# ArtyZe/yolo_quantization

Hardware: AMD Instinct MI355X
Metric: images/sec yolov3-tiny INT8 416x416 (higher is better)
Workload: dtype u8 x s8 -> int32 (f64 or exact-integer requant, bit-identical)

## Files before the change

### include/mi355_yolo_int8.h

```cpp
#ifndef MI355_YOLO_INT8_H
#define MI355_YOLO_INT8_H
#include <stddef.h>
#include <stdint.h>

#ifdef __cplusplus
extern "C" {
#endif

#define MI355_OK 0
#define MI355_EINVAL (-22)
#define MI355_ENOMEM (-12)
#define MI355_EHIP (-5)
#define MI355_ENODEV (-19)

#define MI355_ACT_RELU 1
#define MI355_ACT_LINEAR 3
#define MI355_ACT_RELU6 8
#define MI355_ACT_LEAKY 9

#define MI355_STORE_WRAP 0
#define MI355_STORE_SATURATE 1

#define MI355_ACC_EXACT 0
#define MI355_ACC_REF_F32 1
// ... 38 lines not shown
    int tail;
} mi355_tensor;

size_t mi355_tensor_describe(mi355_tensor *t, int B, int H, int W, int C);
size_t mi355_tensor_describe_nchw(mi355_tensor *t, int B, int H, int W, int C);
int mi355_tensor_fill(const mi355_tensor *t, uint8_t zero_point, void *stream);
int mi355_nchw_to_tensor(const uint8_t *nchw, const mi355_tensor *t, void *stream);
int mi355_tensor_to_nchw(const mi355_tensor *t, uint8_t *nchw, void *stream);

size_t mi355_conv_pack_size(int n, int c, int ksize);
int mi355_conv_pack(int n, int c, int ksize, const uint8_t *weights_uint8, const uint8_t *zp_w,
                    const int32_t *biases_int32, const double *M_value, const double *shift_value, void *blob);
int mi355_conv_pack_epilogue(int n, int c, int ksize, int activation, int zp_act, void *blob);

typedef struct mi355_conv_desc {
    int n, c, ksize, stride, pad;
    int activation;
    int store_mode;
    int accum_mode;
    uint8_t zp_in, zp_act;
    float s_act;
    int plan;
    int epilogue_packed;
} mi355_conv_desc;
#define MI355_PLAN_LATENCY 0
#define MI355_PLAN_THROUGHPUT 1

int mi355_conv_forward(const mi355_conv_desc *desc, const mi355_tensor *x, const void *blob, const uint8_t *w_u8,
                       const uint8_t *zp_w, const mi355_tensor *y, int32_t *acc_out, float *y_f32, void *stream);

int mi355_conv_pool_forward(const mi355_conv_desc *desc, const mi355_tensor *x, const void *blob, const mi355_tensor *y,
                            const mi355_tensor *ypool, void *stream);

int mi355_conv_yolo_forward(const mi355_conv_desc *desc, const mi355_tensor *x, const void *blob, const mi355_tensor *y,
                            float *y_f32, float *yolo_out, int classes, void *stream);

int mi355_conv_upsample_forward(const mi355_conv_desc *desc, const mi355_tensor *x, const void *blob, const mi355_tensor *y_up,
                                int stride, void *stream);

int mi355_conv_shortcut_forward(const mi355_conv_desc *desc, const mi355_tensor *x, const void *blob, const mi355_tensor *from,
                                const mi355_tensor *y_sum, int32_t Ka, int32_t Kb, uint8_t zp_from, uint8_t zp_out, void *stream);

int mi355_conv_forward_per_image(const mi355_conv_desc *desc, const mi355_tensor *x, const void *bank, size_t entry_bytes,
                                 const int32_t *entry_of_image, const uint8_t *zp_in_of_image, const uint8_t *w_u8,
                                 const uint8_t *zp_w, const mi355_tensor *y, int32_t *acc_out, float *y_f32, void *stream);
int mi355_conv_pool_forward_per_image(const mi355_conv_desc *desc, const mi355_tensor *x, const void *bank, size_t entry_bytes,
                                      const int32_t *entry_of_image, const uint8_t *zp_in_of_image, const mi355_tensor *y,
                                      const mi355_tensor *ypool, void *stream);

int mi355_conv_set_tile(int bm, int bn);
int mi355_debug_flags(int flags);
int mi355_last_conv_kernel(void);
int mi355_last_conv_launch(int *grid, int *threads, int *lds_bytes);

int mi355_maxpool_forward(const mi355_tensor *x, const mi355_tensor *y, int size, int stride, int pad, void *stream);
int mi355_upsample_forward(const mi355_tensor *x, const mi355_tensor *y, int stride, void *stream);
int mi355_route_forward(const mi355_tensor *const *xs, int n, const mi355_tensor *y, void *stream);
int mi355_dequant_forward(const mi355_tensor *x, int c0, int nc, uint8_t zero_point, float scale, float *out_f32, int out_C,
                          int out_c0, void *stream);
int mi355_shortcut_multiplier(float s_in, float s_out, int32_t *K);
int mi355_shortcut_forward(const mi355_tensor *a, const mi355_tensor *b, const mi355_tensor *y, int32_t Ka, int32_t Kb,
                           uint8_t zp_a, uint8_t zp_b, uint8_t zp_out, void *stream);
int mi355_letterbox_forward(const float *im_f32, int imw, int imh, int c, float *out_f32, int w, int h, void *stream);
int mi355_image_minmax(const float *x_f32, long count, float *minmax, void *stream);
int mi355_image_quantize(const float *x_f32, long count, float scale, int zero_point, uint8_t *out_u8, void *stream);
int mi355_image_minmax_batched(const float *x_f32, int B, long count_per_image, float *minmax, void *stream);
int mi355_image_quantize_per_image(const float *x_f32, int B, long count_per_image, const float *scale_dev, const uint8_t *zp_dev,
                                   uint8_t *out_u8, void *stream);
#define MI355_INPUT_ALL_ZERO   1u
#define MI355_INPUT_ZERO_SCALE 2u
#define MI355_INPUT_M_RANGE    4u
#define MI355_INPUT_NEG_SHIFT  8u
#define MI355_INPUT_PACK_RANGE 16u
#define MI355_INPUT_BIAS_RANGE 32u
#define MI355_INPUT_BAD_SLOT   64u
typedef struct mi355_l0_channel {
    float bias;
    float w_scale;
    int32_t w_zp;
    int32_t wsum;
} mi355_l0_channel;
typedef struct mi355_l0_consts {
    int32_t n, K;
    int32_t zp_act, activation;
    float s_act;
    int32_t reserved[3];
} mi355_l0_consts;
int mi355_input_pairs(const float *minmax_dev, int B, int shared, int32_t *entry_dev, float *scale_dev, uint8_t *zp_dev,
                      uint32_t *status_dev, void *stream);
int mi355_l0_derive(const mi355_l0_consts *consts_dev, const mi355_l0_consts *consts_host, void *bank, size_t entry_bytes, int B,
                    int shared, float *scale_dev, uint8_t *zp_dev, float *kept_scale_dev, uint8_t *kept_zp_dev, uint32_t *status_dev,
                    void *stream);
#define MI355_FRAME_RGB 0
#define MI355_FRAME_BGR 1
typedef struct mi355_frame_u8 {
    const uint8_t *data;
    int w, h;
    int pitch;
    int order;
    int reserved[2];
} mi355_frame_u8;
int mi355_frames_u8_letterbox_minmax(const mi355_frame_u8 *table_dev, const mi355_frame_u8 *table_host, int B, int w, int h,
                                     float *minmax, void *stream);
int mi355_frames_u8_letterbox_quantize(const mi355_frame_u8 *table_dev, const mi355_frame_u8 *table_host, int B, int w, int h,
                                       const float *scale_dev, const uint8_t *zp_dev, uint8_t *out_u8, void *stream);
#define MI355_YUV_NV12 0
// ... 170 lines not shown
```

### yolo_quantization_amd/binding.py

```python
from __future__ import annotations

import ctypes as C
import os

import numpy as np

_HERE = os.path.dirname(os.path.abspath(__file__))
LIB_DIR = os.environ.get("MI355_LIB_DIR") or os.path.join(_HERE, "lib")

ACT = {"relu": 1, "linear": 3, "relu6": 8, "leaky": 9}
STORE_WRAP, STORE_SATURATE = 0, 1
ACC_EXACT, ACC_REF_F32 = 0, 1


class MI355Error(RuntimeError):
    pass


class Tensor(C.Structure):
    _fields_ = [("data", C.c_void_p), ("B", C.c_int), ("H", C.c_int), ("W", C.c_int), ("C", C.c_int),
                ("cs", C.c_int), ("lead", C.c_int), ("tail", C.c_int)]


class ConvDesc(C.Structure):
# ... 263 lines not shown


class DevTensor:

    def __init__(self, B, H, W, Cc, zero_point=0):
        self.t = Tensor()
        nbytes = shim().mi355_tensor_describe(C.byref(self.t), B, H, W, Cc)
        if not nbytes:
            raise MI355Error("bad tensor dims")
        self.buf = DevBuf(nbytes)
        self.t.data = self.buf.ptr
        check(shim().mi355_tensor_fill(C.byref(self.t), zero_point, None), "fill")

    @classmethod
    def from_nchw(cls, x, zero_point=0):
        x = np.ascontiguousarray(x, np.uint8)
        B, Cc, H, W = x.shape
        t = cls(B, H, W, Cc, zero_point)
        src = DevBuf.from_numpy(x)
        check(shim().mi355_nchw_to_tensor(src.ptr, C.byref(t.t), None), "nchw_to_tensor")
        check(shim().mi355_stream_sync(None), "sync")
        return t

    def to_nchw(self):
        n = self.t.B * self.t.C * self.t.H * self.t.W
        dst = DevBuf(n)
        check(shim().mi355_tensor_to_nchw(C.byref(self.t), dst.ptr, None), "tensor_to_nchw")
        return dst.to_numpy(np.uint8, n).reshape(self.t.B, self.t.C, self.t.H, self.t.W)

    def ref(self):
        return C.byref(self.t)


def conv_pack(wq, zp_w, c, ksize, biases_int32, M_value, shift_value, activation=None, zp_act=None, pad=None):
    wq = np.ascontiguousarray(wq, np.uint8)
    n = wq.shape[0]
    sz = shim().mi355_conv_pack_size(n, c, ksize)
    if not sz:
        raise MI355Error(f"unsupported conv shape n={n} c={c} k={ksize}")
    blob = np.zeros(sz, np.uint8)
    zp_w = np.ascontiguousarray(zp_w, np.uint8)
    b = np.ascontiguousarray(biases_int32, np.int32)
    mv = np.ascontiguousarray(M_value, np.float64)
    sv = np.ascontiguousarray(shift_value, np.float64)
    check(shim().mi355_conv_pack(n, c, ksize, wq.ctypes.data, zp_w.ctypes.data, b.ctypes.data, mv.ctypes.data,
                                 sv.ctypes.data, blob.ctypes.data), "conv_pack")
    if activation is not None:
        check(shim().mi355_conv_pack_epilogue(n, c, ksize, int(activation), int(zp_act), blob.ctypes.data), "conv_pack_epilogue")
    return blob


def last_conv_kernel():
    return int(shim().mi355_last_conv_kernel())


def last_conv_launch():
    g, t, l = C.c_int(), C.c_int(), C.c_int()
    shim().mi355_last_conv_launch(C.byref(g), C.byref(t), C.byref(l))
    return g.value, t.value, l.value


def _pack_blob(wq, zp_w, c, ksize, biases_int32, M_value, shift_value, activation, zp_act, epilogue):
    ept = (activation, zp_act) if epilogue else ()
    return DevBuf.from_numpy(conv_pack(wq, zp_w, c, ksize, biases_int32, M_value, shift_value, *ept))


def conv_forward(x: DevTensor, wq, zp_w, ksize, biases_int32, M_value, shift_value, zp_in, zp_act, s_act,
                 activation, store=STORE_WRAP, accum=ACC_EXACT, want_acc=True, want_f32=False, stride=1, pad=None,
                 plan=0, epilogue=False):
    n = wq.shape[0]
    c = x.t.C
    blob = _pack_blob(wq, zp_w, c, ksize, biases_int32, M_value, shift_value, activation, zp_act, epilogue)
    wraw = DevBuf.from_numpy(np.ascontiguousarray(wq, np.uint8))
    zraw = DevBuf.from_numpy(np.ascontiguousarray(zp_w, np.uint8))
    if pad is None:
        pad = ksize // 2
    OH, OW = (x.t.H + 2 * pad - ksize) // stride + 1, (x.t.W + 2 * pad - ksize) // stride + 1
    y = DevTensor(x.t.B, OH, OW, n, zp_act)
    cnt = x.t.B * n * OH * OW
    acc = DevBuf(cnt * 4) if want_acc else None
    f32 = DevBuf(cnt * 4) if want_f32 else None
    d = ConvDesc(n, c, ksize, stride, pad, activation, store, accum, zp_in, zp_act, float(s_act), int(plan), int(bool(epilogue)))
    check(shim().mi355_conv_forward(C.byref(d), x.ref(), blob.ptr, wraw.ptr, zraw.ptr, y.ref(),
                                    acc.ptr if acc else None, f32.ptr if f32 else None, None), "conv_forward")
    check(shim().mi355_stream_sync(None), "sync")
    out = {"u8": y.to_nchw(), "tensor": y}
    if acc:
        out["int32"] = acc.to_numpy(np.int32, cnt).reshape(x.t.B, n, OH * OW)
    if f32:
        out["f32"] = f32.to_numpy(np.float32, cnt).reshape(x.t.B, n, OH * OW)
    return out


FUSED = ("pool2", "pool1", "upsample", "yolo", "shortcut")


def conv_fused_forward(x: DevTensor, wq, zp_w, ksize, biases_int32, M_value, shift_value, zp_in, zp_act, s_act, activation, fuse,
                       store=STORE_WRAP, plan=0, epilogue=False, keep_y=False, classes=80, up=2, res=None, Ka=0, Kb=0,
                       zp_from=0, zp_out=0):
    assert fuse in FUSED, fuse
    n = wq.shape[0]
    c = x.t.C
    B, H, W = x.t.B, x.t.H, x.t.W
    blob = _pack_blob(wq, zp_w, c, ksize, biases_int32, M_value, shift_value, activation, zp_act, epilogue)
    d = ConvDesc(n, c, ksize, 1, ksize // 2, activation, store, ACC_EXACT, zp_in, zp_act, float(s_act), int(plan), int(bool(epilogue)))
    S = shim()
# ... 983 lines not shown
```

### yolo_quantization_amd/csrc/conv_rows.hip

```cpp
#include "kargs.h"
#include <type_traits>

#if defined(MI355_ABLATE) && !defined(ROWS_TU_KS1)
#define DBG(bit) ((a.debug & (bit)) != 0)
#define TS_PHASES 6
#define TS_BLOCKS 4096
__device__ long long g_rows_ts[TS_PHASES][TS_BLOCKS];
#define TS(k)                                                                                   \
    do {                                                                                        \
        if (threadIdx.x == 0 && blockIdx.x < TS_BLOCKS) g_rows_ts[k][blockIdx.x] = wall_clock64(); \
    } while (0)
extern "C" int mi355_debug_read_ts(long long *host)
{
    return hipMemcpyFromSymbol(host, HIP_SYMBOL(g_rows_ts), sizeof(long long) * TS_PHASES * TS_BLOCKS) == hipSuccess ? 0 : -5;
}
#define WP_PHASES 5
__device__ long long g_rows_wp[TS_BLOCKS][8][WP_PHASES];
#define WP_DECL long long wp_acc[WP_PHASES] = {0, 0, 0, 0, 0}; long long wp_t = 0
#define WP_START()                                                   \
    do {                                                             \
        if (DBG(256)) { wp_t = __builtin_readcyclecounter(); }       \
    } while (0)
#define WP_MARK(k)                                                   \
    do {                                                             \
        if (DBG(256)) {                                              \
            asm volatile("s_waitcnt lgkmcnt(0)" ::: "memory");       \
            const long long wp_n = __builtin_readcyclecounter();     \
            wp_acc[k] += wp_n - wp_t;                                \
            wp_t = wp_n;                                             \
        }                                                            \
    } while (0)
#define WP_FLUSH()                                                                                   \
    do {                                                                                             \
        if (DBG(256) && lane == 0 && blockIdx.x < TS_BLOCKS && wave < 8)                             \
            for (int k = 0; k < WP_PHASES; ++k) g_rows_wp[blockIdx.x][wave][k] = wp_acc[k];          \
    } while (0)
extern "C" int mi355_debug_read_wp(long long *host)
{
    return hipMemcpyFromSymbol(host, HIP_SYMBOL(g_rows_wp), sizeof(long long) * TS_BLOCKS * 8 * WP_PHASES) == hipSuccess ? 0 : -5;
}
#else
#define DBG(bit) (false)
#define TS(k) do { } while (0)
#define WP_DECL do { } while (0)
#define WP_START() do { } while (0)
#define WP_MARK(k) do { } while (0)
#define WP_FLUSH() do { } while (0)
#endif

#define DMA16(gsrc, ldst)                                                                               \
    __builtin_amdgcn_global_load_lds((const __attribute__((address_space(1))) void *)(gsrc),           \
                                     (__attribute__((address_space(3))) void *)(ldst), 16, 0, 0)

template <int KS, int BN> constexpr int ra_stages() { return KS == 3 ? (BN <= 192 ? 4 : 6) : (BN <= 128 ? 4 : 3); }
template <int KS, int BN> constexpr int rb_stages() { return KS == 3 ? 2 : ra_stages<KS, BN>(); }
constexpr int rows_nb_slots(int BN, int RS, int NW, int KS)
{
    const int wmin = RS * 3 / 4, halo = KS == 3 ? 1 : 0;
    const int rows = (BN - 2 + wmin) / wmin + 1 + (BN - 2 + wmin * wmin) / (wmin * wmin) + 2 * halo;
    return (rows * (RS / 16) + NW - 1) / NW;
}

__device__ __forceinline__ void row_of_pixel(int n, int H, int W, FastDiv fd_hw, FastDiv fd_w, int &grow, int &x)
{
    const int hw = H * W;
    const int b = fd_div(n, fd_hw);
    const int r = n - b * hw;
    const int y = fd_div(r, fd_w);
    x = r - y * W;
    grow = b * (H + 1) + y + 1;
}

template <int BM, int BN, int WMW, int WNW, int RS, int KS>
__global__ __launch_bounds__(64 * WMW * WNW, 2) void conv_rows_i8_kernel(const ConvArgs a)
{
    constexpr int NW = WMW * WNW, NT = 64 * NW;
    constexpr int TM = BM / WMW, TN = BN / WNW;
    constexpr int MS = TM / 32, NS = TN / 32;
    constexpr int ACH = BM / 16;
    constexpr int DW = (NW == 8 && KS == 3) ? 4 : NW;
    constexpr int APT = (ACH + DW - 1) / DW;
    constexpr int HALO = (KS == 3) ? 1 : 0;
    constexpr int PIECEB = RS * 16;
    constexpr int CPR = RS / 16;
    constexpr int OSTR = BM + 4;
    constexpr int RA_STAGES = ra_stages<KS, BN>();
    constexpr int RB_STAGES = rb_stages<KS, BN>();
    constexpr int NBS = rows_nb_slots(BN, RS, DW, KS);
    constexpr int SPS = (NBS + 3) / 4;
    static_assert(TM % 32 == 0 && TN % 32 == 0, "wave tile must be a multiple of the 32x32 MFMA tile");

    extern __shared__ __attribute__((aligned(16))) char smem[];
    char *ldsA = smem;
    char *ldsB = smem + RA_STAGES * BM * 64;
    const int rowb = a.rowb;
    const int bbytes = a.rows_cap * rowb;
    int *ldsS = reinterpret_cast<int *>(ldsB + RB_STAGES * bbytes);
    double *ldsPM = reinterpret_cast<double *>(smem + a.lds_param_off);
    int *ldsPI = reinterpret_cast<int *>(ldsPM + 3 * BM);
    float *ldsYL = reinterpret_cast<float *>(ldsPI + 2 * BM);

    const int tid = threadIdx.x;
    const int lane = tid & 63;
    const int wave = __builtin_amdgcn_readfirstlane(tid >> 6);
    const int wm = wave / WNW, wn = wave % WNW;
    const int kh = lane >> 5, lj = lane & 31;
    const int dwave = wave & (DW - 1);
    const bool issuer = wave < DW;
    TS(0);

    int logical;
    {
        const int nb = gridDim.x, id = blockIdx.x;
        const int q = nb >> 3, r = nb & 7, xcd = id & 7, idx = id >> 3;
        logical = (xcd < r ? xcd * (q + 1) : r * (q + 1) + (xcd - r) * q) + idx;
    }
    int mtile, ntile;
    {
        const int blk = fd_div(logical, a.fd_ntper);
        const int rem = logical - blk * (a.xcd_mb * a.ntiles_n);
        ntile = fd_div(rem, a.fd_mb);
        mtile = blk * a.xcd_mb + (rem - ntile * a.xcd_mb);
    }
    const int n0 = ntile * a.tile_q + min(ntile, a.tile_r);
    const int n_end = n0 + a.tile_q + (ntile < a.tile_r ? 1 : 0);
    const int W1 = a.W + 1, hw = a.H * a.W;

    int gr0, x0;
// ... 59 lines not shown
        const int j = min(dwave + i * DW, ndma - 1);
        const int r = j / CPR, cj = j - r * CPR;
        const int o = cj * 1024 + lane * 16;
        const int p = o / PIECEB, c = (o - p * PIECEB) >> 4;
        long f = cell0 + (long)r * W1 + c;
        f = f < 0 ? 0 : (f > a.in_cells - 1 ? a.in_cells - 1 : f);
        bvoff[i] = (unsigned)(f * a.in_cs + p * 16);
        bdst[i] = lds0 + RA_STAGES * BM * 64 + r * rowb + (cj << 10);
    }
    auto issueB_slots = [&](int chunk, auto lo_c, auto hi_c) {
        constexpr int LO = decltype(lo_c)::value, HI = decltype(hi_c)::value;
        if (DW < NW && !issuer) return;
        const unsigned boff = (chunk % RB_STAGES) * bbytes;
        int phys = chunk + rot;
        if (phys >= a.nchunks) phys -= a.nchunks;
        const int8_t *base = a.x + (size_t)phys * 64;
#pragma unroll
        for (int i = LO; i < HI; ++i) {
            const unsigned d = bdst[i] + boff, v = bvoff[i];
            DMA_S(d, base, v);
        }
    };
    auto issueB = [&](int chunk) { issueB_slots(chunk, std::integral_constant<int, 0>{}, std::integral_constant<int, NBS>{}); };

    TS(1);
    if constexpr (KS == 3) {
        issueB(0);
#pragma unroll
        for (int st = 0; st < RA_STAGES - 1; ++st) issueA_next(st * (BM * 64));
    } else {
#pragma unroll
        for (int st = 0; st < RA_STAGES - 1; ++st)
            if (st < a.ksteps) {
                issueB(st);
                issueA_next(st * (BM * 64));
            }
    }

    v16i acc[MS][NS];
#pragma unroll
    for (int ms = 0; ms < MS; ++ms)
#pragma unroll
        for (int grp = 0; grp < 4; ++grp) {
            const int4 c4 = *reinterpret_cast<const int4 *>(a.cwb + mtile * BM + wm * TM + ms * 32 + 8 * grp + 4 * kh);
#pragma unroll
            for (int ns = 0; ns < NS; ++ns) {
                acc[ms][ns][grp * 4 + 0] = c4.x;
                acc[ms][ns][grp * 4 + 1] = c4.y;
                acc[ms][ns][grp * 4 + 2] = c4.z;
                acc[ms][ns][grp * 4 + 3] = c4.w;
            }
        }

    for (int i = tid; i < a.rows_cap * RS; i += NT) ldsS[i] = 0;
    if (a.yolo_out)
        for (int i = tid; i < 256; i += NT) ldsYL[i] = yolo_entry_act((float)(i - a.zp_act) * a.s_act, 0);
    for (int i = tid; i < BM; i += NT) {
        const int oc = mtile * BM + i;
        ldsPM[i] = a.mval[oc];
        ldsPM[BM + i] = a.sval[oc];
        ldsPI[i] = a.dzp[oc];
        ldsPI[BM + i] = a.bias[oc];
        ldsPM[2 * BM + i] = a.mprime[oc];
    }

    int sxr[NS];
#pragma unroll
    for (int ns = 0; ns < NS; ++ns) sxr[ns] = 0;
    auto compute = [&](const char *A, const char *Bt, int tapoff) {
#pragma unroll
        for (int h = 0; h < 2; ++h) {
            v4i af[MS];
#pragma unroll
            for (int ms = 0; ms < MS; ++ms) af[ms] = *reinterpret_cast<const v4i *>(A + atab[ms] + h * 512);
#pragma unroll
            for (int ns = 0; ns < NS; ++ns) {
                const v4i bf = *reinterpret_cast<const v4i *>(Bt + bbase[ns] + tapoff + h * 2 * PIECEB);
                int t = sxr[ns];
                t = __builtin_amdgcn_sdot4(bf[0], 0x01010101, t, false);
                t = __builtin_amdgcn_sdot4(bf[1], 0x01010101, t, false);
                t = __builtin_amdgcn_sdot4(bf[2], 0x01010101, t, false);
                t = __builtin_amdgcn_sdot4(bf[3], 0x01010101, t, false);
                sxr[ns] = t;
#pragma unroll
                for (int ms = 0; ms < MS; ++ms)
                    acc[ms][ns] = __builtin_amdgcn_mfma_i32_32x32x32_i8(af[ms], bf, acc[ms][ns], 0, 0, 0);
            }
        }
    };
    auto cell_sums = [&](const char *Bt) {
        const int ncells = nrows * RS;
        for (int id = tid; id < ncells; id += NT) {
            const int r = id / RS, c = id - r * RS;
            const char *p0 = Bt + r * rowb + c * 16;
            int t = 0;
#pragma unroll
            for (int p = 0; p < 4; ++p) {
                const v4i v = *reinterpret_cast<const v4i *>(p0 + p * PIECEB);
                t = __builtin_amdgcn_sdot4(v[0], 0x01010101, t, false);
                t = __builtin_amdgcn_sdot4(v[1], 0x01010101, t, false);
                t = __builtin_amdgcn_sdot4(v[2], 0x01010101, t, false);
                t = __builtin_amdgcn_sdot4(v[3], 0x01010101, t, false);
            }
            ldsS[id] += t;
        }
    };

    if constexpr (KS == 3) {
        constexpr int R = RA_STAGES;
        static_assert(R == 6 || R == 4, "ring depths the stage bookkeeping below is written for");
        constexpr int ROT = 9 % R;
        v4i fa[3][MS], fb[3][NS];
        unsigned aaddr[R][MS], baddr[3][NS];
#pragma unroll
        for (int st = 0; st < R; ++st)
#pragma unroll
            for (int ms = 0; ms < MS; ++ms) aaddr[st][ms] = lds0 + st * (BM * 64) + atab[ms];
#pragma unroll
        for (int ty = 0; ty < 3; ++ty)
#pragma unroll
            for (int ns = 0; ns < NS; ++ns) baddr[ty][ns] = lds0 + R * BM * 64 + bbase[ns] + ty * rowb;
#define LDS_READ128(dst, addr, imm) asm volatile("ds_read_b128 %0, %1 offset:%2" : "=v"(dst) : "v"(addr), "n"(imm))
        auto half = [&](const v4i(&ca)[MS], const v4i(&cb)[NS], v4i(&na)[MS], v4i(&nb)[NS], const unsigned(&aad)[MS],
                        const unsigned(&bad)[NS], auto tap_c, auto h_c, auto rd_c, auto prev_rd_c, auto &&hook) {
            constexpr int TAPOFF = decltype(tap_c)::value, H = decltype(h_c)::value;
            constexpr bool RD = decltype(rd_c)::value, PREV_RD = decltype(prev_rd_c)::value;
            const bool rd = RD && !DBG(8);
            if (PREV_RD) asm volatile("s_waitcnt lgkmcnt(%0)" ::"n"(MS + NS) : "memory");
            else asm volatile("s_waitcnt lgkmcnt(0)" ::: "memory");
            __builtin_amdgcn_sched_barrier(0);
            if (!DBG(4)) acc[0][0] = __builtin_amdgcn_mfma_i32_32x32x32_i8(ca[0], cb[0], acc[0][0], 0, 0, 0);
            __builtin_amdgcn_sched_barrier(0);
            hook();
            if (rd) {
#pragma unroll
                for (int ms = 0; ms < MS; ++ms) LDS_READ128(na[ms], aad[ms], H * 512);
            }
            __builtin_amdgcn_sched_barrier(0);
            if (MS > 1 && !DBG(4)) acc[MS - 1][0] = __builtin_amdgcn_mfma_i32_32x32x32_i8(ca[MS - 1], cb[0], acc[MS - 1][0], 0, 0, 0);
            __builtin_amdgcn_sched_barrier(0);
            if (rd) {
                LDS_READ128(nb[0], bad[0], TAPOFF + H * 2 * PIECEB);
                if (NS > 1) LDS_READ128(nb[NS > 1 ? 1 : 0], bad[NS > 1 ? 1 : 0], TAPOFF + H * 2 * PIECEB);
            }
            __builtin_amdgcn_sched_barrier(0);
#pragma unroll
            for (int ns = 1; ns < NS; ++ns) {
                if (!DBG(4)) {
#pragma unroll
                    for (int ms = 0; ms < MS; ++ms)
                        acc[ms][ns] = __builtin_amdgcn_mfma_i32_32x32x32_i8(ca[ms], cb[ns], acc[ms][ns], 0, 0, 0);
                }
                __builtin_amdgcn_sched_barrier(0);
                if (ns + 1 < NS && rd) LDS_READ128(nb[ns + 1 < NS ? ns + 1 : 0], bad[ns + 1 < NS ? ns + 1 : 0], TAPOFF + H * 2 * PIECEB);
                __builtin_amdgcn_sched_barrier(0);
            }
        };
        auto nohook = [] {};
        using std::integral_constant;
        using std::true_type;
        using std::false_type;
        asm volatile("s_waitcnt vmcnt(%0)" ::"n"((R - 3) * APT) : "memory");
        __builtin_amdgcn_s_barrier();
        TS(2);
#pragma unroll
        for (int ms = 0; ms < MS; ++ms) LDS_READ128(fa[0][ms], aaddr[0][ms], 0);
#pragma unroll
        for (int ns = 0; ns < NS; ++ns) LDS_READ128(fb[0][ns], baddr[0][ns], 0);
#pragma unroll
        for (int ms = 0; ms < MS; ++ms) LDS_READ128(fa[1][ms], aaddr[0][ms], 512);
#pragma unroll
        for (int ns = 0; ns < NS; ++ns) LDS_READ128(fb[1][ns], baddr[0][ns], 2 * PIECEB);
        WP_DECL;
        WP_START();
        auto chunk_body = [&](auto last_c, int chunk) {
            constexpr bool LAST = decltype(last_c)::value;
            const char *Bt = ldsB + (chunk & 1) * bbytes;
            const bool odd = chunk & 1;
            auto step = [&](auto t_c) {
                constexpr int t = decltype(t_c)::value;
                constexpr int TYN = ((t + 1) % 9) / 3;
                constexpr int TAPN = ((t + 1) % 3) * 16;
                constexpr int SN = (t == 8) ? 0 : (t + 1) % R;
                constexpr int C0 = (2 * t) % 3, C1 = (2 * t + 1) % 3, N0 = (2 * t + 2) % 3, N1 = (2 * t + 3) % 3;
                constexpr bool RD = (t < 8) || !LAST;
                constexpr bool ISSUE_A = !LAST || (t + R - 1 < 9);
                constexpr auto n_b = [](int st) { return (LAST || st < 0 || st >= 4) ? 0 : ((st + 1) * SPS < NBS ? (st + 1) * SPS : NBS) - (st * SPS < NBS ? st * SPS : NBS); };
                constexpr auto n_a = [](int st) { return (st < 0 || !LAST || st + R - 1 < 9) ? APT : 0; };
                constexpr int YOUNG = n_a(t - 1) + n_b(t - 1) + (R > 4 ? n_a(t - 2) + n_b(t - 2) + n_a(t - 3) + n_b(t - 3) : 0);
                constexpr int BLO = t * SPS < NBS ? t * SPS : NBS, BHI = (t + 1) * SPS < NBS ? (t + 1) * SPS : NBS;
                if (t == 8 && !LAST) {
                    const int bdelta = odd ? -bbytes : bbytes;
                    unsigned rot[R][MS];
#pragma unroll
                    for (int st = 0; st < R; ++st)
#pragma unroll
                        for (int ms = 0; ms < MS; ++ms) rot[st][ms] = aaddr[(st + ROT) % R][ms];
#pragma unroll
                    for (int st = 0; st < R; ++st)
#pragma unroll
                        for (int ms = 0; ms < MS; ++ms) aaddr[st][ms] = rot[st][ms];
#pragma unroll
                    for (int yy = 0; yy < 3; ++yy)
#pragma unroll
                        for (int ns = 0; ns < NS; ++ns) baddr[yy][ns] += bdelta;
                }
                WP_MARK(0);
                if (t > 0 || chunk > 0) {
                    asm volatile("s_waitcnt vmcnt(%0)" ::"n"(YOUNG) : "memory");
                    WP_MARK(1);
                    if (!DBG(2)) __builtin_amdgcn_s_barrier();
                    WP_MARK(2);
                }
                half(fa[C0], fb[C0], fa[N0], fb[N0], aaddr[SN], baddr[TYN], integral_constant<int, TAPN>{},
                     integral_constant<int, 0>{}, integral_constant<bool, RD>{}, true_type{}, [&] {
                         if (!LAST && t < 4 && !DBG(1))
                             issueB_slots(chunk + 1, integral_constant<int, BLO>{}, integral_constant<int, BHI>{});
                         if (ISSUE_A && !DBG(1)) {
                             if constexpr (R == 6) {
                                 constexpr unsigned E = ((t + R - 1) % R) * (BM * 64), O = ((t + R - 1 + 3) % R) * (BM * 64);
                                 issueA_next(odd ? O : E);
                             } else {
                                 issueA_next((unsigned)((chunk + t + R - 1) & 3) * (BM * 64));
                             }
                         }
                     });
                WP_MARK(3);
                half(fa[C1], fb[C1], fa[N1], fb[N1], aaddr[SN], baddr[TYN], integral_constant<int, TAPN>{},
                     integral_constant<int, 1>{}, integral_constant<bool, RD>{}, integral_constant<bool, RD>{}, nohook);
                WP_MARK(4);
                if (t == 1 && !DBG(16)) {
                    asm volatile("s_waitcnt lgkmcnt(0)" ::: "memory");
                    cell_sums(Bt);
                    asm volatile("s_waitcnt lgkmcnt(0)" ::: "memory");
                    __builtin_amdgcn_sched_barrier(0);
                }
            };
            step(integral_constant<int, 0>{}); step(integral_constant<int, 1>{}); step(integral_constant<int, 2>{});
            step(integral_constant<int, 3>{}); step(integral_constant<int, 4>{}); step(integral_constant<int, 5>{});
            step(integral_constant<int, 6>{}); step(integral_constant<int, 7>{}); step(integral_constant<int, 8>{});
        };
        for (int chunk = 0; chunk + 1 < a.nchunks; ++chunk) chunk_body(false_type{}, chunk);
        chunk_body(true_type{}, a.nchunks - 1);
        asm volatile("s_waitcnt lgkmcnt(0)" ::: "memory");
        WP_FLUSH();
#undef LDS_READ128
    } else {
        TS(2);
        constexpr int R1 = RA_STAGES;
        constexpr int G = NBS + APT;
        static_assert(RB_STAGES == R1 && (R1 == 3 || R1 == 4), "1x1 loop: common ring depth");
        for (int g0 = 0; g0 < a.ksteps; g0 += R1) {
#pragma unroll
            for (int u = 0; u < R1; ++u) {
                const int g = g0 + u;
                if (g < a.ksteps) {
                    const int young = min(R1 - 2, a.ksteps - 1 - g);
                    if (young == R1 - 2) asm volatile("s_waitcnt vmcnt(%0)" ::"n"((R1 - 2) * G) : "memory");
                    else if (young == 1) asm volatile("s_waitcnt vmcnt(%0)" ::"n"(G) : "memory");
                    else asm volatile("s_waitcnt vmcnt(0)" ::: "memory");
                    __builtin_amdgcn_s_barrier();
                    if (g + R1 - 1 < a.ksteps) {
                        issueB(g + R1 - 1);
                        issueA_next(((u + R1 - 1) % R1) * (BM * 64));
                    }
                    const char *Bt = ldsB + u * bbytes;
                    compute(ldsA + u * (BM * 64), Bt, 0);
                    __builtin_amdgcn_sched_barrier(0);
                }
            }
        }
    }

    TS(3);
    if (DBG(32)) {
        if (acc[0][0][0] == 0x7fffffff && a.y) a.y[tid] = 1;
        return;
    }
    __syncthreads();
    int sx[NS];
#pragma unroll
    for (int ns = 0; ns < NS; ++ns) {
        int t = 0;
        if (KS == 1) {
            t = sxr[ns] + __shfl_xor(sxr[ns], 32);
        } else {
            const int c0 = prow[ns] * RS + pcol[ns];
#pragma unroll
            for (int dy = 0; dy < KS; ++dy)
#pragma unroll
                for (int dx = 0; dx < KS; ++dx) t += ldsS[c0 + dy * RS + dx];
        }
        sx[ns] = t;
    }
    __syncthreads();
    char *otile = smem;
    int *celltab = reinterpret_cast<int *>(smem + BN * OSTR);
// ... 133 lines not shown
    }
#endif
    __syncthreads();
    TS(4);
    if (a.y && !DBG(128)) {
        const int dwords = min(BM, a.out_w - m0) >> 2;
        if (a.up > 1) {
            const int total = BN * dwords, rowc = a.up * a.W + 1;
            for (int p = tid; p < total; p += NT) {
                const int pix = p / dwords, d = p - pix * dwords;
                const int cell = celltab[pix];
                if (cell >= 0) {
                    const uint32_t v = *reinterpret_cast<const uint32_t *>(otile + pix * OSTR + d * 4);
                    for (int uy = 0; uy < a.up; ++uy)
                        for (int ux = 0; ux < a.up; ++ux)
                            *reinterpret_cast<uint32_t *>(a.y + (size_t)(cell + uy * rowc + ux) * a.out_cs + m0 + d * 4) = v;
                }
            }
        } else if (dwords == BM / 4 && !(a.out_cs & 15) && !((size_t)a.y & 15)) {
#pragma unroll 2
            for (int p = tid; p < BN * (BM / 16); p += NT) {
                const int pix = p / (BM / 16), q = p % (BM / 16);
                const int cell = celltab[pix];
                if (cell >= 0) {
                    const uint32_t *sp = reinterpret_cast<const uint32_t *>(otile + pix * OSTR + q * 16);
                    const uint4 v = make_uint4(sp[0], sp[1], sp[2], sp[3]);
                    *reinterpret_cast<uint4 *>(a.y + (size_t)cell * a.out_cs + m0 + q * 16) = v;
                }
            }
        } else if (dwords == BM / 4) {
#pragma unroll 4
            for (int p = tid; p < BN * (BM / 4); p += NT) {
                const int pix = p / (BM / 4), d = p % (BM / 4);
                const int cell = celltab[pix];
                if (cell >= 0)
                    *reinterpret_cast<uint32_t *>(a.y + (size_t)cell * a.out_cs + m0 + d * 4) =
                        *reinterpret_cast<const uint32_t *>(otile + pix * OSTR + d * 4);
            }
        } else {
            const int total = BN * dwords;
            for (int p = tid; p < total; p += NT) {
                const int pix = p / dwords, d = p - pix * dwords;
                const int cell = celltab[pix];
                if (cell >= 0)
                    *reinterpret_cast<uint32_t *>(a.y + (size_t)cell * a.out_cs + m0 + d * 4) =
                        *reinterpret_cast<const uint32_t *>(otile + pix * OSTR + d * 4);
            }
        }
    }
    TS(5);
}

template <int BM, int BN, int WMW, int WNW, int RS, int KS>
static int rows_launch_cfg(ConvArgs &a, hipStream_t st)
{
    constexpr int NW = WMW * WNW, NT = 64 * NW;
    constexpr int DW = (NW == 8 && KS == 3) ? 4 : NW;
    constexpr int HALO = (KS == 3) ? 1 : 0;
    if (a.mpad % BM) return MI355_EINVAL;
    a.mtiles = a.mpad / BM;
    if (a.ntiles_n < (a.total_n + BN - 1) / BN) a.ntiles_n = (a.total_n + BN - 1) / BN;
    a.rows_cap = (BN - 2 + a.W) / a.W + 1 + (BN - 2 + a.H * a.W) / (a.H * a.W) + 2 * HALO;
    const int ndma = a.rows_cap * (RS / 16);
    if ((ndma + DW - 1) / DW > rows_nb_slots(BN, RS, DW, KS)) return MI355_EINVAL;
    if ((size_t)a.in_cells * (size_t)a.in_cs >= ((size_t)1 << 32)) return MI355_EINVAL;
    a.rowb = RS * 64 + 16 * (a.W & 15);
    a.fd_hw = fastdiv_make((uint32_t)(a.H * a.W)); a.fd_w = fastdiv_make((uint32_t)a.W);
    a.fd_ntn = fastdiv_make((uint32_t)a.ntiles_n); a.fd_nch = fastdiv_make((uint32_t)a.nchunks);
    a.tile_q = a.total_n / a.ntiles_n; a.tile_r = a.total_n % a.ntiles_n;
    size_t lds = (size_t)ra_stages<KS, BN>() * BM * 64 + (size_t)rb_stages<KS, BN>() * a.rows_cap * a.rowb + (size_t)a.rows_cap * RS * 4;
    const size_t lds_epi = (size_t)BN * (BM + 4) + (size_t)BN * 4;
    if (lds_epi > lds) lds = lds_epi;
    lds = (lds + 15) & ~(size_t)15;
    a.lds_param_off = (int)lds;
    lds += (size_t)BM * 32 + (a.yolo_out ? 1024 : 0);
    if (lds > 160 * 1024) return MI355_EINVAL;
    auto kern = conv_rows_i8_kernel<BM, BN, WMW, WNW, RS, KS>;
    static size_t lds_attr_dev[64] = {0};
    int dev_ix = 0;
    (void)hipGetDevice(&dev_ix);
    size_t &lds_attr = lds_attr_dev[dev_ix & 63];
    if (lds > 64 * 1024 && lds > lds_attr) {
        lds_attr = lds;
        if (hipFuncSetAttribute(reinterpret_cast<const void *>(kern), hipFuncAttributeMaxDynamicSharedMemorySize,
                                (int)lds) != hipSuccess)
            return MI355_EHIP;
    }
    a.xcd_mb = 1;
    if (!(a.debug & (1 << 24))) {
        const long nb = (long)a.ntiles_n * a.mtiles, per = (nb + 7) / 8;
        const double wslab = (double)BM * a.ksteps * 64, itile = (double)a.total_n / a.ntiles_n * a.cb * a.nchunks;
        double best = 0;
        for (int mb = 1; mb <= a.mtiles; ++mb) {
            if (a.mtiles % mb) continue;
            const long blk = (long)mb * a.ntiles_n;
            const long mt = std::min<long>(a.mtiles, mb * ((per + blk - 1) / blk)), nt = std::min<long>(a.ntiles_n, (per + mb - 1) / mb + (per % mb || blk % per || nb % 8 ? 1 : 0));
            const double bytes = mt * wslab + nt * itile;
            if (mb == 1 || bytes < best) { best = bytes; a.xcd_mb = mb; }
        }
    }
    a.fd_ntper = fastdiv_make((uint32_t)(a.xcd_mb * a.ntiles_n));
    a.fd_mb = fastdiv_make((uint32_t)a.xcd_mb);
    dim3 grid(a.ntiles_n * a.mtiles), block(NT);
    conv_launch_note(grid.x, NT, lds);
    hipLaunchKernelGGL(kern, grid, block, lds, st, a);
    return hipGetLastError() == hipSuccess ? MI355_OK : MI355_EHIP;
}

template <int RS, int KS>
static int rows_launch_tile(ConvArgs &a, hipStream_t st, int bm, int bn)
{
    if (bm == 128 && bn == 384) return rows_launch_cfg<128, 384, 2, 4, RS, KS>(a, st);
    if (bm == 128 && bn == 256) return rows_launch_cfg<128, 256, 2, 4, RS, KS>(a, st);
    if constexpr (KS == 3) {
        if (bm == 128 && bn == 192) return rows_launch_cfg<128, 192, 2, 2, RS, KS>(a, st);
    }
    if (bm == 128 && bn == 128) return rows_launch_cfg<128, 128, 2, 2, RS, KS>(a, st);
    if (bm == 64 && bn == 256) return rows_launch_cfg<64, 256, 1, 4, RS, KS>(a, st);
    if (bm == 64 && bn == 128) return rows_launch_cfg<64, 128, 1, 4, RS, KS>(a, st);
    if (bm == 32 && bn == 256) return rows_launch_cfg<32, 256, 1, 4, RS, KS>(a, st);
    if (bm == 32 && bn == 128) return rows_launch_cfg<32, 128, 1, 4, RS, KS>(a, st);
    return MI355_EINVAL;
}

#ifdef ROWS_TU_KS1
int conv_rows_launch_k1(ConvArgs &a, hipStream_t st, int bm, int bn)
{
    const int need = a.W + 2;
    if (need <= 16) return rows_launch_tile<16, 1>(a, st, bm, bn);
    if (need <= 32) return rows_launch_tile<32, 1>(a, st, bm, bn);
    if (need <= 64) return rows_launch_tile<64, 1>(a, st, bm, bn);
    return MI355_EINVAL;
}
#else
int conv_rows_launch_k1(ConvArgs &a, hipStream_t st, int bm, int bn);

int conv_rows16_launch(ConvArgs &a, hipStream_t st, int bm, int bn);

int conv_rows_launch(ConvArgs &a, hipStream_t st, int bm, int bn)
{
    if (a.cb != 64) return MI355_EINVAL;
    if (a.ksize != 3) return conv_rows_launch_k1(a, st, bm, bn);
    if (!(a.debug & (1 << 20))) {
        const int rc = conv_rows16_launch(a, st, bm, bn);
        if (rc != MI355_EINVAL) return rc;
    }
    const int need = a.W + 2;
    if (need <= 16) return rows_launch_tile<16, 3>(a, st, bm, bn);
    if (need <= 32) return rows_launch_tile<32, 3>(a, st, bm, bn);
    if (need <= 64) return rows_launch_tile<64, 3>(a, st, bm, bn);
    return MI355_EINVAL;
}
#endif
```

### yolo_quantization_amd/csrc/kargs.h

```cpp
#pragma once
#include "common.h"
#include <atomic>
#include <type_traits>
#include <mutex>

struct ConvArgs {
    const int8_t *x;
    const int8_t *wp;
    const int32_t *cw, *dzp, *bias;
    const double *mval, *sval;
    uint8_t *y;
    int32_t *acc_out;
    float *y_f32;
    int in_cs, in_lead, in_cells;
    int out_cs, out_lead;
    int out_w, pool_w;
    int B, H, W, n;
    int stride, OH, OW;
    int ksize, cb, nchunks, upc, spc, ksteps;
    int total_n, ntiles_n, mtiles;
    int xcd_mb;
    FastDiv fd_hw, fd_w, fd_ntn, fd_ntper, fd_nch, fd_mb;
    int tile_q, tile_r;
    int zp_act, act, store_mode;
    float s_act;
    int mpad;
    int bchunks, bpt;
    int tiles_x, tiles_y;
    int rows_cap;
    int rowb;
    const int32_t *shift;
    const double *mprime;
    const int32_t *cwb;
    const ConvBlobHeader *hdr;
    uint8_t *ypool;
    int pool_cs, pool_lead;
    int lds_param_off;
    int debug;
    const int8_t *ws;
    int sm_ncell, sm_pieceb;
    int sm_lcell, sm_hc;
    int sm_tp;
    int sm_nq, sm_red_off;
    int pool_mode;
    int sm_pt_off, sm_pt_stride;
    int up;
    float *yolo_out;
    int yolo_per;
    const uint8_t *res;
    int res_cs, res_delta;
    int sc_ka, sc_kb, sc_k0;
    int plan;
    const EptHeader *ept;
};

struct AuxArgs {
    const uint8_t *x;
    int in_cs, in_lead, in_cells;
    const uint32_t *wfirst;
    const uint8_t *w_u8;
    const uint8_t *zp_w;
    const int32_t *dzp, *bias;
    const double *mval, *sval;
    uint8_t *y;
    int out_cs, out_lead;
    int32_t *acc_out;
    float *y_f32;
    int B, H, W, c, n, ksize, pad;
    int zp_in, zp_act, act, store_mode;
    float s_act;
    int total_n;
    const double *mprime;
    uint8_t *ypool;
    int pool_cs, pool_lead;
    const ConvBlobHeader *hdr;
    const int32_t *cwb;
    int planar;
    int debug_flags;
    const EptHeader *ept;
    FastDiv fd_tpi, fd_tx;
    const int32_t *entry_of_image;
    const uint8_t *zp_of_image;
    long entry_bytes;
    int pi_wpi;
};

template <bool PI>
__device__ __forceinline__ std::conditional_t<PI, AuxArgs, const AuxArgs &> bank_entry(const AuxArgs &a, int b)
{
    if constexpr (!PI) {
        return a;
    } else {
        AuxArgs e = a;
        const long off = (long)a.entry_of_image[b] * a.entry_bytes;
        auto mv = [off](auto *p) { return p ? reinterpret_cast<decltype(p)>(reinterpret_cast<const char *>(p) + off) : p; };
        e.wfirst = mv(a.wfirst); e.dzp = mv(a.dzp); e.bias = mv(a.bias);
        e.mval = mv(a.mval); e.sval = mv(a.sval); e.mprime = mv(a.mprime);
        e.hdr = mv(a.hdr); e.cwb = mv(a.cwb); e.ept = mv(a.ept);
        e.zp_in = a.zp_of_image[b];
        return e;
    }
}

struct PoolArgs {
    const uint8_t *x;
    uint8_t *y;
// ... 31 lines not shown
struct KxkArgs {
    const uint8_t *x;
    int in_cs, in_lead;
    int B, H, W, c;
    int n, ksize, stride, pad, OH, OW;
    const int8_t *wk;
    int unit, nchunks, spc, ksteps;
    const int32_t *cw, *dzp, *bias, *cwb;
    const double *mval, *sval, *mprime;
    const ConvBlobHeader *hdr;
    const uint8_t *w_u8, *zp_w;
    uint8_t *y;
    int out_cs, out_lead;
    int32_t *acc_out;
    float *y_f32;
    int zp_in, zp_act, act, store_mode;
    float s_act;
    int tw_sh, tiles_x, tiles_y, mgroups, ph, pw;
};
int conv_kxk_launch(KxkArgs &a, hipStream_t st);
int conv_ref_f32_general_launch(KxkArgs &a, hipStream_t st);
inline int kxk_unit(int c) { return c <= 4 ? 4 : (c <= 8 ? 8 : 16); }
struct KxkGeom { int unit, nchunks, spc, ksteps, mpad; };
inline KxkGeom kxk_geom(int n, int c, int ksize)
{
    KxkGeom g;
    g.unit = kxk_unit(c);
    const int tpl = 16 / g.unit;
    g.nchunks = g.unit == 16 ? (c + 15) / 16 : 1;
    g.spc = (ksize * ksize + 2 * tpl - 1) / (2 * tpl);
    g.ksteps = g.nchunks * g.spc;
    g.mpad = ((n + 127) / 128) * 128;
    return g;
}

int yolo_detections_launch(const float *out, int B, int n, int classes, int h, int w, const float *biases, const int *mask,
                           int netw, int neth, int imw, int imh, float thresh, int relative, float *recs, int max_recs,
                           int *counts, hipStream_t st);
int conv_igemm_launch(ConvArgs &a, hipStream_t st);
int conv_rows_launch(ConvArgs &a, hipStream_t st, int bm, int bn);
int conv_small_pool_launch(ConvArgs &a, hipStream_t st);
__host__ __device__ constexpr int ws_row_filter(int R) { return 16 * ((R >> 2) & 1) + 4 * (R >> 3) + (R & 3); }
bool conv_small_eligible(int n, int c, int ksize);
bool conv_pool16_eligible(int n, int c, int ksize);
int conv_pool16_launch(ConvArgs &a, hipStream_t st);
bool conv_small32_eligible(int n, int c, int ksize);
int conv_small32_launch(ConvArgs &a, hipStream_t st);
int conv1x1_ws_launch(ConvArgs &a, hipStream_t st);
bool conv1x1_ws_eligible(int n, int c, int ksize);
int conv_ws3_launch(ConvArgs &a, hipStream_t st);
bool conv_ws3_eligible(int n, int c, int ksize);
int mi355_debug_flags_get();
void conv_launch_note(long grid, int threads, size_t lds);
static inline bool plan_one_round(const ConvArgs &a)
{
    const int rs = a.W + 2 <= 16 ? 16 : (a.W + 2 <= 32 ? 32 : 64);
    return a.plan == MI355_PLAN_THROUGHPUT && (long)((a.mpad + 127) / 128) * ((a.total_n + 383) / 384) <= 256 && 10 * (a.W + 2) >= 7 * rs;
}
int conv_first_launch(AuxArgs &a, hipStream_t st);
int conv_first_pool_launch(AuxArgs &a, hipStream_t st);
int conv_first_mfma_pool_launch(AuxArgs &a, hipStream_t st);
int conv_first_mfma_launch(AuxArgs &a, hipStream_t st);
int conv_ref_f32_launch(AuxArgs &a, hipStream_t st);
int maxpool_launch(const PoolArgs &a, hipStream_t st);
int copy_cells_launch(const CopyArgs &a, hipStream_t st);
int copy_cell_bytes_launch(const CopyArgs &a, int nbytes, hipStream_t st);
int nchw_to_phwc_launch(const LayoutArgs &a, hipStream_t st);
int phwc_to_nchw_launch(const LayoutArgs &a, hipStream_t st);
int dequant_cells_launch(const DequantArgs &a, hipStream_t st);
int shortcut_launch(const ShortcutArgs &a, hipStream_t st);
int fill_u32_launch(uint32_t *p, uint32_t v, long n, hipStream_t st);
int letterbox_launch(const float *im, int imw, int imh, int c, float *out, int w, int h, hipStream_t st);
int image_minmax_launch(const float *x, long count, uint32_t *mm, hipStream_t st);
int image_quantize_launch(const float *x, long count, float scale, int zp, uint8_t *out, hipStream_t st);
int image_minmax_batched_launch(const float *x, int B, long count, uint32_t *mm, hipStream_t st);
int image_quantize_per_image_launch(const float *x, int B, long count, const float *scale_dev, const uint8_t *zp_dev, uint8_t *out,
                                    hipStream_t st);
int image_minmax_seed_launch(uint32_t *mm, int B, hipStream_t st);
int input_pairs_launch(const float *mm, int B, int shared, int32_t *entry, float *scale, uint8_t *zp, uint32_t *status, hipStream_t st);
int l0_derive_launch(const mi355_l0_consts *consts, int activation, void *bank, long entry_bytes, int B, int shared, float *scale, uint8_t *zp,
                     float *kept_scale, uint8_t *kept_zp, uint32_t *status, hipStream_t st);
struct SourceU8;
struct SourceYUV;
struct SourcePlanar;
struct SourcePacked;
struct SourceP010;
struct SourceBayer;
template <class Source, class Frame> const char *frames_check(const Frame *host, int B, int w, int h);
template <class Source, class Frame> int frames_letterbox_minmax_launch(const Frame *table_dev, int B, int w, int h, uint32_t *mm, hipStream_t st);
template <class Source, class Frame>
int frames_letterbox_quantize_launch(const Frame *table_dev, int B, int w, int h, const float *scale_dev, const uint8_t *zp_dev, uint8_t *out,
                                     hipStream_t st);
const char *jpeg_idct_check(const mi355_jpeg_plane *host, int nplanes);
int jpeg_idct_launch(const mi355_jpeg_plane *table_dev, const mi355_jpeg_plane *table_host, int nplanes, hipStream_t st);
const char *jpeg_to_rgb_check(const mi355_jpeg_image *host, int B);
int jpeg_to_rgb_launch(const mi355_jpeg_image *table_dev, const mi355_jpeg_image *table_host, int B, hipStream_t st);
const char *jpeg_entropy_check(const mi355_jpeg_segment *host, int nsegments, int subseq_bits);
int jpeg_entropy_launch(const mi355_jpeg_segment *table_dev, int nsegments, int subseq_bits, int *status_dev, hipStream_t st);
int yolo_detections_sizes_launch(const float *out, int B, int n, int classes, int h, int w, const float *biases, const int *mask,
                                 int netw, int neth, const int *imw_dev, const int *imh_dev, float thresh, int relative, float *recs,
                                 int max_recs, int *counts, hipStream_t st);
int yolo_logistic_launch(const float *in, float *out, int B, int n, int classes, int hw, hipStream_t st);
struct DetHead {
    const float *out, *biases;
    const int *mask;
    int n, h, w;
// ... 40 lines not shown
```

### yolo_quantization_amd/csrc/shim.hip

```cpp
#include "kargs.h"
#include <chrono>
#include <mutex>
#include <stdio.h>
#include <string.h>
#include <stdlib.h>
#include <math.h>


static thread_local char g_err[512] = "";
static int hip_fail(hipError_t e, const char *what)
{
    snprintf(g_err, sizeof(g_err), "%s: %s", what, hipGetErrorString(e));
    return MI355_EHIP;
}
#define HIPCHK(call)                                      \
    do {                                                  \
        hipError_t e__ = (call);                          \
        if (e__ != hipSuccess) return hip_fail(e__, #call); \
    } while (0)
static int einval(const char *msg)
{
    snprintf(g_err, sizeof(g_err), "invalid argument: %s", msg);
    return MI355_EINVAL;
}
// ... 245 lines not shown
    return (size_t)t->lead + (size_t)t->B * (t->H + 1) * (t->W + 1) + t->tail;
}

size_t mi355_tensor_describe(mi355_tensor *t, int B, int H, int W, int C)
{
    if (!t || B <= 0 || H <= 0 || W <= 0 || C <= 0) return 0;
    t->B = B; t->H = H; t->W = W; t->C = C;
    t->cs = (C == 3) ? 4 : ((C + 15) / 16) * 16;
    t->lead = 2;
    t->tail = W + 3;
    return tensor_cells(t) * (size_t)t->cs;
}

size_t mi355_tensor_describe_nchw(mi355_tensor *t, int B, int H, int W, int C)
{
    if (!t || B <= 0 || H <= 0 || W <= 0 || C <= 0) return 0;
    t->B = B; t->H = H; t->W = W; t->C = C;
    t->cs = 1; t->lead = 0; t->tail = 0;
    return (size_t)B * C * H * W;
}

int mi355_tensor_fill(const mi355_tensor *t, uint8_t zero_point, void *stream)
{
    if (!t || !t->data) return einval("tensor");
    if (t->cs == 1) return einval("tensor_fill: a planar tensor has no pad cells");
    const size_t cells = tensor_cells(t);
    if (t->cs == 4) {
        const uint32_t v = (uint32_t)zero_point | ((uint32_t)zero_point << 8) | ((uint32_t)zero_point << 16);
        return fill_u32_launch((uint32_t *)t->data, v, (long)cells, (hipStream_t)stream);
    }
    HIPCHK(hipMemsetAsync(t->data, zero_point ^ 0x80, cells * t->cs, (hipStream_t)stream));
    return MI355_OK;
}

int mi355_nchw_to_tensor(const uint8_t *nchw, const mi355_tensor *t, void *stream)
{
    if (!nchw || !t || !t->data) return einval("nchw_to_tensor");
    LayoutArgs a{const_cast<uint8_t *>(nchw), (uint8_t *)t->data, t->B, t->H, t->W, t->C, t->cs, t->lead};
    return nchw_to_phwc_launch(a, (hipStream_t)stream);
}
int mi355_tensor_to_nchw(const mi355_tensor *t, uint8_t *nchw, void *stream)
{
    if (!nchw || !t || !t->data) return einval("tensor_to_nchw");
    LayoutArgs a{nchw, (uint8_t *)t->data, t->B, t->H, t->W, t->C, t->cs, t->lead};
    return phwc_to_nchw_launch(a, (hipStream_t)stream);
}

static int default_bm(int n) { return n >= 128 ? 128 : (n > 32 ? 64 : 32); }
static size_t align16(size_t v) { return (v + 15) & ~(size_t)15; }

static thread_local int g_last_kernel = 0;
extern "C" int mi355_last_conv_kernel(void) { return g_last_kernel; }
static thread_local long g_last_grid = 0;
static thread_local int g_last_threads = 0, g_last_lds = 0;
extern "C++" void conv_launch_note(long grid, int threads, size_t lds)
{
    g_last_grid = grid; g_last_threads = threads; g_last_lds = (int)lds;
}
extern "C" int mi355_last_conv_launch(int *grid, int *threads, int *lds_bytes)
{
    if (grid) *grid = (int)g_last_grid;
    if (threads) *threads = g_last_threads;
    if (lds_bytes) *lds_bytes = g_last_lds;
    return g_last_grid ? MI355_OK : MI355_EINVAL;
}

static bool specialised_shape(int c, int ksize) { return (ksize == 1 || ksize == 3) && ((c == 3 && ksize == 3) || c % 16 == 0); }

static int blob_layout(int n, int c, int ksize, ConvBlobHeader *h)
{
    if (n <= 0 || c <= 0 || ksize < 1 || ksize > 11) return MI355_EINVAL;
    memset(h, 0, sizeof(*h));
    h->magic = MI355_BLOB_MAGIC;
    h->n = n; h->c = c; h->ksize = ksize;
    h->ktrue = c * ksize * ksize;
    size_t off = align16(sizeof(ConvBlobHeader));
    const KxkGeom kg = kxk_geom(n, c, ksize);
    const size_t gen_bytes = (size_t)(kg.mpad / 32) * kg.ksteps * 1024;
    if (!specialised_shape(c, ksize)) {
        h->generic = 1;
        h->mpad = kg.mpad;
        h->cb = kg.unit;
        h->nchunks = kg.nchunks;
        h->upc = ksize * ksize;
        h->spc = kg.spc;
        h->ksteps = kg.ksteps;
        h->off_wp = off; h->off_gen = off; off = align16(off + gen_bytes);
    } else if (c == 3 && ksize == 3) {
        h->first = 1;
        h->mpad = ((n + 3) / 4) * 4;
        h->cb = 4; h->nchunks = 1; h->upc = 9; h->spc = 9; h->ksteps = 9;
        h->off_wp = off; off = align16(off + (size_t)h->mpad * 9 * 4);
    } else {
        if (c % 16) return MI355_EINVAL;
        const int bm = default_bm(n);
        h->mpad = ((n + bm - 1) / bm) * bm;
        h->cb = (c % 64 == 0) ? 64 : (c % 32 == 0 ? 32 : 16);
        h->nchunks = c / h->cb;
        h->upc = ksize * ksize * (h->cb / 16);
        h->spc = (h->upc + 3) / 4;
        h->ksteps = h->nchunks * h->spc;
        h->off_wp = off; off = align16(off + (size_t)h->mpad * h->ksteps * 64);
    }
    h->off_cw = off;   off = align16(off + (size_t)h->mpad * 4);
    h->off_dzp = off;  off = align16(off + (size_t)h->mpad * 4);
    h->off_bias = off; off = align16(off + (size_t)h->mpad * 4);
    h->off_mval = off; off = align16(off + (size_t)h->mpad * 8);
    h->off_sval = off; off = align16(off + (size_t)h->mpad * 8);
    h->off_shift = off; off = align16(off + (size_t)h->mpad * 4);
    h->off_mprime = off; off = align16(off + (size_t)h->mpad * 8);
    h->off_cwb = off; off = align16(off + (size_t)h->mpad * 4);
// ... 853 lines not shown
```

Before: 280,100.

## Add cell-ownership variant of 3x3 rows kernel interleaving cell sums with MMA

Adds a templated OWN form of the rows conv kernel for 128x128 tiles with RS=32 and 3x3 kernels. In it each thread owns one input cell and accumulates that cell's zero-point sum with sdot4 during the k-halves of the main loop, instead of a separate cell_sums pass with lgkmcnt waits at t==1. The per-thread sums are written to LDS at the end, and the LDS zeroing is skipped. The form is chosen at launch when rows_cap*(W+2) fits in the thread count. This adds extra LDS reads and registers inside the hot loop and a fastdiv argument.

```diff
diff --git a/include/mi355_yolo_int8.h b/include/mi355_yolo_int8.h
--- a/include/mi355_yolo_int8.h
+++ b/include/mi355_yolo_int8.h
@@ -114,6 +114,7 @@
 int mi355_debug_flags(int flags);
 int mi355_last_conv_kernel(void);
 int mi355_last_conv_launch(int *grid, int *threads, int *lds_bytes);
+int mi355_last_conv_form(void);
 
 int mi355_maxpool_forward(const mi355_tensor *x, const mi355_tensor *y, int size, int stride, int pad, void *stream);
 int mi355_upsample_forward(const mi355_tensor *x, const mi355_tensor *y, int stride, void *stream);
diff --git a/yolo_quantization_amd/binding.py b/yolo_quantization_amd/binding.py
--- a/yolo_quantization_amd/binding.py
+++ b/yolo_quantization_amd/binding.py
@@ -339,6 +339,10 @@
 
 def last_conv_kernel():
     return int(shim().mi355_last_conv_kernel())
+
+
+def last_conv_form():
+    return int(shim().mi355_last_conv_form())
 
 
 def last_conv_launch():
diff --git a/yolo_quantization_amd/csrc/conv_rows.hip b/yolo_quantization_amd/csrc/conv_rows.hip
--- a/yolo_quantization_amd/csrc/conv_rows.hip
+++ b/yolo_quantization_amd/csrc/conv_rows.hip
@@ -71,9 +71,10 @@
     grow = b * (H + 1) + y + 1;
 }
 
-template <int BM, int BN, int WMW, int WNW, int RS, int KS>
-__global__ __launch_bounds__(64 * WMW * WNW, 2) void conv_rows_i8_kernel(const ConvArgs a)
-{
+template <int BM, int BN, int WMW, int WNW, int RS, int KS, bool OWN>
+__device__ __forceinline__ void rows_tile(const ConvArgs &a)
+{
+    static_assert(!OWN || KS == 3, "cell ownership is a form of the 3x3 loop");
     constexpr int NW = WMW * WNW, NT = 64 * NW;
     constexpr int TM = BM / WMW, TN = BN / WNW;
     constexpr int MS = TM / 32, NS = TN / 32;
@@ -239,7 +240,8 @@
             }
         }
 
-    for (int i = tid; i < a.rows_cap * RS; i += NT) ldsS[i] = 0;
+    if constexpr (!OWN)
+        for (int i = tid; i < a.rows_cap * RS; i += NT) ldsS[i] = 0;
     if (a.yolo_out)
         for (int i = tid; i < 256; i += NT) ldsYL[i] = yolo_entry_act((float)(i - a.zp_act) * a.s_act, 0);
     for (int i = tid; i < BM; i += NT) {
@@ -343,7 +345,14 @@
                 __builtin_amdgcn_sched_barrier(0);
             }
         };
-        auto nohook = [] {};
+        int csum = 0;
+        unsigned caddr = 0;
+        v4i cv;
+        if constexpr (OWN) {
+            const int cid = tid < nrows * (a.W + 2) ? tid : 0;
+            const int r = fd_div(cid, a.fd_w2), c = cid - r * (a.W + 2);
+            caddr = lds0 + R * BM * 64 + r * rowb + c * 16;
+        }
         using std::integral_constant;
         using std::true_type;
         using std::false_type;
@@ -376,8 +385,27 @@
                 constexpr auto n_a = [](int st) { return (st < 0 || !LAST || st + R - 1 < 9) ? APT : 0; };
                 constexpr int YOUNG = n_a(t - 1) + n_b(t - 1) + (R > 4 ? n_a(t - 2) + n_b(t - 2) + n_a(t - 3) + n_b(t - 3) : 0);
                 constexpr int BLO = t * SPS < NBS ? t * SPS : NBS, BHI = (t + 1) * SPS < NBS ? (t + 1) * SPS : NBS;
+                constexpr auto cs_piece = [](int q) { return OWN && q >= 0 && q < 16 && q % 4 == 0 ? q / 4 : -1; };
+                static_assert(cs_piece(16) < 0 && cs_piece(17) < 0, "cell reads ride on k-halves that read fragments");
+                auto cell_piece = [&](auto q_c) {
+                    constexpr int q = decltype(q_c)::value;
+                    if constexpr (cs_piece(q - 1) >= 0) {
+                        if (!DBG(16)) {
+                            csum = __builtin_amdgcn_sdot4(cv[0], 0x01010101, csum, false);
+                            csum = __builtin_amdgcn_sdot4(cv[1], 0x01010101, csum, false);
+                            csum = __builtin_amdgcn_sdot4(cv[2], 0x01010101, csum, false);
+                            csum = __builtin_amdgcn_sdot4(cv[3], 0x01010101, csum, false);
+                        }
+                        __builtin_amdgcn_sched_barrier(0);
+                    }
+                    if constexpr (cs_piece(q) >= 0) {
+                        const unsigned ca = caddr;
+                        if (!DBG(16)) LDS_READ128(cv, ca, cs_piece(q) * PIECEB);
+                    }
+                };
                 if (t == 8 && !LAST) {
                     const int bdelta = odd ? -bbytes : bbytes;
+                    if constexpr (OWN) caddr += bdelta;
                     unsigned rot[R][MS];
 #pragma unroll
                     for (int st = 0; st < R; ++st)
@@ -411,12 +439,15 @@
                                  issueA_next((unsigned)((chunk + t + R - 1) & 3) * (BM * 64));
                              }
                          }
+                         cell_piece(integral_constant<int, 2 * t>{});
                      });
                 WP_MARK(3);
                 half(fa[C1], fb[C1], fa[N1], fb[N1], aaddr[SN], baddr[TYN], integral_constant<int, TAPN>{},
-                     integral_constant<int, 1>{}, integral_constant<bool, RD>{}, integral_constant<bool, RD>{}, nohook);
+                     integral_constant<int, 1>{}, integral_constant<bool, RD>{}, integral_constant<bool, RD>{}, [&] {
+                         cell_piece(integral_constant<int, 2 * t + 1>{});
+                     });
                 WP_MARK(4);
-                if (t == 1 && !DBG(16)) {
+                if (!OWN && t == 1 && !DBG(16)) {
                     asm volatile("s_waitcnt lgkmcnt(0)" ::: "memory");
                     cell_sums(Bt);
                     asm volatile("s_waitcnt lgkmcnt(0)" ::: "memory");
@@ -430,6 +461,12 @@
         for (int chunk = 0; chunk + 1 < a.nchunks; ++chunk) chunk_body(false_type{}, chunk);
         chunk_body(true_type{}, a.nchunks - 1);
         asm volatile("s_waitcnt lgkmcnt(0)" ::: "memory");
+        if constexpr (OWN) {
+            if (tid < nrows * (a.W + 2)) {
+                const int r = fd_div(tid, a.fd_w2);
+                ldsS[r * RS + tid - r * (a.W + 2)] = csum;
+            }
+        }
         WP_FLUSH();
 #undef LDS_READ128
     } else {
@@ -669,6 +706,20 @@
 }
 
 template <int BM, int BN, int WMW, int WNW, int RS, int KS>
+__global__ __launch_bounds__(64 * WMW * WNW, 2) void conv_rows_i8_kernel(const ConvArgs a)
+{
+    rows_tile<BM, BN, WMW, WNW, RS, KS, false>(a);
+}
+
+template <int BM, int BN, int WMW, int WNW, int RS, int KS>
+__global__ __launch_bounds__(64 * WMW * WNW, 2) void conv_rows_i8_kernel_own(const ConvArgs a)
+{
+    rows_tile<BM, BN, WMW, WNW, RS, KS, true>(a);
+}
+
+template <int BM, int BN, int RS, int KS> constexpr bool rows_has_own() { return KS == 3 && BM == 128 && BN == 128 && RS == 32; }
+
+template <int BM, int BN, int WMW, int WNW, int RS, int KS>
 static int rows_launch_cfg(ConvArgs &a, hipStream_t st)
 {
     constexpr int NW = WMW * WNW, NT = 64 * NW;
@@ -692,11 +743,19 @@
     a.lds_param_off = (int)lds;
     lds += (size_t)BM * 32 + (a.yolo_out ? 1024 : 0);
     if (lds > 160 * 1024) return MI355_EINVAL;
-    auto kern = conv_rows_i8_kernel<BM, BN, WMW, WNW, RS, KS>;
-    static size_t lds_attr_dev[64] = {0};
+    void (*kern)(const ConvArgs) = conv_rows_i8_kernel<BM, BN, WMW, WNW, RS, KS>;
+    bool own = false;
+    if constexpr (rows_has_own<BM, BN, RS, KS>()) {
+        own = a.rows_cap * (a.W + 2) <= NT && !(a.debug & (1 << 30));
+        if (own) {
+            a.fd_w2 = fastdiv_make((uint32_t)(a.W + 2));
+            kern = conv_rows_i8_kernel_own<BM, BN, WMW, WNW, RS, KS>;
+        }
+    }
+    static size_t lds_attr_dev[2][64] = {{0}};
     int dev_ix = 0;
     (void)hipGetDevice(&dev_ix);
-    size_t &lds_attr = lds_attr_dev[dev_ix & 63];
+    size_t &lds_attr = lds_attr_dev[own][dev_ix & 63];
     if (lds > 64 * 1024 && lds > lds_attr) {
         lds_attr = lds;
         if (hipFuncSetAttribute(reinterpret_cast<const void *>(kern), hipFuncAttributeMaxDynamicSharedMemorySize,
@@ -720,6 +779,7 @@
     a.fd_mb = fastdiv_make((uint32_t)a.xcd_mb);
     dim3 grid(a.ntiles_n * a.mtiles), block(NT);
     conv_launch_note(grid.x, NT, lds);
+    conv_launch_form(own ? 1 : 0);
     hipLaunchKernelGGL(kern, grid, block, lds, st, a);
     return hipGetLastError() == hipSuccess ? MI355_OK : MI355_EHIP;
 }
diff --git a/yolo_quantization_amd/csrc/kargs.h b/yolo_quantization_amd/csrc/kargs.h
--- a/yolo_quantization_amd/csrc/kargs.h
+++ b/yolo_quantization_amd/csrc/kargs.h
@@ -52,6 +52,7 @@
     int sc_ka, sc_kb, sc_k0;
     int plan;
     const EptHeader *ept;
+    FastDiv fd_w2;
 };
 
 struct AuxArgs {
@@ -189,6 +190,7 @@
 bool conv_ws3_eligible(int n, int c, int ksize);
 int mi355_debug_flags_get();
 void conv_launch_note(long grid, int threads, size_t lds);
+void conv_launch_form(int form);
 static inline bool plan_one_round(const ConvArgs &a)
 {
     const int rs = a.W + 2 <= 16 ? 16 : (a.W + 2 <= 32 ? 32 : 64);
diff --git a/yolo_quantization_amd/csrc/shim.hip b/yolo_quantization_amd/csrc/shim.hip
--- a/yolo_quantization_amd/csrc/shim.hip
+++ b/yolo_quantization_amd/csrc/shim.hip
@@ -321,11 +321,14 @@
 static thread_local int g_last_kernel = 0;
 extern "C" int mi355_last_conv_kernel(void) { return g_last_kernel; }
 static thread_local long g_last_grid = 0;
-static thread_local int g_last_threads = 0, g_last_lds = 0;
+static thread_local int g_last_threads = 0, g_last_lds = 0, g_last_form = 0;
 extern "C++" void conv_launch_note(long grid, int threads, size_t lds)
 {
     g_last_grid = grid; g_last_threads = threads; g_last_lds = (int)lds;
-}
+    g_last_form = 0;
+}
+extern "C++" void conv_launch_form(int form) { g_last_form = form; }
+extern "C" int mi355_last_conv_form(void) { return g_last_form; }
 extern "C" int mi355_last_conv_launch(int *grid, int *threads, int *lds_bytes)
 {
     if (grid) *grid = (int)g_last_grid;
```

New measurement: 279,800. No clear change (-0.1%).
